# cviviers/graph-physics

Hardware: AMD Instinct MI355X
Metric: training-steps/sec + one-step velocity MSE, CylinderFlow MGN 15MP h=128 (higher is better)
Workload: dtype bf16; 1 GPU; CylinderFlow MGN 15MP h=128, batch=8 graphs per GPU (Cfg B); nodes_per_gpu=15384, edges_per_gpu=88560, global_batch=8, parallelism=dp1

## Files before the change

### graph-physics_amd/csrc/mgn_chain.h

```cpp
#pragma once
#include "mgn_common.h"

struct ChainFwdArgs {
    const __bf16* e;
    const __bf16* proj;
    const int32_t* proj_i;
    const int32_t* proj_j;
    const __bf16* wpack;
    int64_t woff[4];
    int32_t wks[4];
    const float* bias[4];
    const float* scale;
    float dinv;
    int64_t M, ntiles;
    __bf16* out;
    __bf16* z_save;
    float* rden_save;
    __bf16* act8;
    int64_t act_off[4];
    unsigned* mask32;
    int64_t mask_stride;
    float* agg_full;
    float* agg_head;
    float* agg_tail;
// ... 61 lines not shown
    float* rden_save;
    __bf16* act8;
    int64_t act_off[4];
    unsigned* mask32;
    int64_t mask_stride;
    const __bf16* pn_pack;
    const float* pn_b0;
    __bf16* pn_out;
    int32_t pn_kst;
    const float* agg_full;
    const float* agg_head;
    const float* agg_tail;
};

struct ChainNodeBwdArgs {
    const __bf16* dout;
    const __bf16* z_save;
    const float* rden_save;
    const float* scale;
    float dinv;
    const unsigned* mask32;
    int64_t mask_stride;
    const __bf16* wtpack;
    int64_t woff[4];
    int32_t wks[4];
    int64_t M, ntiles;
    __bf16* dz8;
    int64_t RP;
    float* dscale_part;
    __bf16* dx_part;
    __bf16* d_aggr;
};

bool chain_eligible(const mgn_mlp* m);
int chain16_edge_backward_parts(int64_t M);
int chain16_node_backward_parts(int64_t M);
bool chain_node_eligible(const mgn_mlp* m);
int chain16_node_forward(const mgn_mlp* m, const void* x, const mgn_topology* t, const mgn_mlp* edge,
                         const mgn_mlp_saved* edge_sv, int64_t M, void* x_out, void* aggr_save, mgn_mlp_saved* sv,
                         hipStream_t st, const mgn_mlp* next_edge = nullptr, void* next_proj = nullptr,
                         void* agg_scratch = nullptr);
size_t chain16_edge_agg_bytes(int64_t N, int64_t E);
int chain16_node_backward(const mgn_mlp* m, int64_t M, const mgn_mlp_saved* sv, const void* dout, void* dz8,
                          float* dscale_part, int* nparts, void* dx_part, void* d_aggr, hipStream_t st,
                          bool din2 = false);
int chain16_edge_forward(const mgn_mlp* m, const void* e, const void* proj, const int32_t* pi, const int32_t* pj,
                         int64_t M, void* out, mgn_mlp_saved* sv, hipStream_t st, bool z_p2, bool save_act = true,
                         int64_t N = 0, void* agg_scratch = nullptr);
int chain16_edge_wgrad_recompute(const mgn_mlp* m, const void* e, const void* proj, const int32_t* pi, const int32_t* pj,
                                 int64_t M, const void* dz8, float* part, int64_t G, int rows_per_chunk, int nchunks,
                                 hipStream_t st);
int chain16_edge_backward(const mgn_mlp* m, int64_t M, const mgn_mlp_saved* sv, const void* dout, const void* gath,
                          const int32_t* gath_idx, void* dz8, float* dscale_part, int* nparts, void* de, void* dz0,
                          hipStream_t st, bool p2, bool din2 = false, bool dout2 = false, int64_t N = 0,
                          void* agg_scratch = nullptr);
void chain16_edge_agg_parts(void* scratch, int64_t N, int64_t E, float** full, float** head, float** tail);
bool chain_dense_eligible(const mgn_mlp* m);
int chain16_dense_forward(const mgn_mlp* m, const void* in, int in_dtype, int64_t in_ld, const int32_t* in_rows,
                          int64_t M, void* out, int out_dtype, mgn_mlp_saved* sv, hipStream_t st);
int chain16_dense_backward(const mgn_mlp* m, int64_t M, const mgn_mlp_saved* sv, const void* dout, int dout_dtype,
                           void* din, int din_dtype, int64_t din_ld, void* dz8, float* dscale_part, int* nparts,
                           hipStream_t st);
```

### graph-physics_amd/csrc/mgn_chain16.hip

```cpp
#include <cmath>
#include <utility>
#include <cstring>
#include <mutex>
#include <type_traits>

#include "mgn_chain.h"
#include "mgn_chain16_dev.h"

#ifndef MGN_ABLATE
#define MGN_ABLATE 0
#endif
#ifndef MGN_DIRECT_ROWS
#define MGN_DIRECT_ROWS 0
#endif


#ifndef MGN_PROJ_HANDOFF
#define MGN_PROJ_HANDOFF 1
#endif

#ifndef MGN_BWD_HANDOFF
#define MGN_BWD_HANDOFF 1
#endif

// ... 1457 lines not shown
            relu_mask(acc, mcur[l - 1]);
            to_operand(acc, B);
        }
        store_r8(acc, scr, a.dz8, tile, lane);
        if (a.din) {
            f4 d2[2] = {f4{0.f, 0.f, 0.f, 0.f}, f4{0.f, 0.f, 0.f, 0.f}};
#pragma unroll
            for (int s = 0; s < 4; ++s)
#pragma unroll
                for (int t = 0; t < 2; ++t) d2[t] = mfma16(wfrag(W, 0, t, s, lane), B[s], d2[t]);
            if (ok) {
#pragma unroll
                for (int t = 0; t < 2; ++t)
#pragma unroll
                    for (int r = 0; r < 4; ++r) {
                        const int k = 16 * t + 4 * g + r;
                        if (k < a.K0) {
                            if (a.din_f32)
                                reinterpret_cast<float*>(a.din)[row * a.din_ld + k] = d2[t][r];
                            else
                                reinterpret_cast<__bf16*>(a.din)[row * a.din_ld + k] = (__bf16)d2[t][r];
                        }
                    }
            }
        }
        dpin<F32D>(nxt);
    }
    __syncthreads();
    if (threadIdx.x < H) {
        float s = 0.f;
#pragma unroll
        for (int w = 0; w < NW; ++w) s += red[w * H + threadIdx.x];
        a.dscale_part[(int64_t)blockIdx.x * H + threadIdx.x] = s;
    }
}

}

static size_t agg_al(size_t x) { return (x + 255) & ~(size_t)255; }
size_t chain16_edge_agg_bytes(int64_t N, int64_t E) {
    const int64_t nt = rows_pad(E) / TR;
    return agg_al((size_t)N * H * 4) + 2 * agg_al((size_t)nt * H * 4);
}
static void agg_carve(void* scratch, int64_t N, int64_t E, float** full, float** head, float** tail) {
    char* p = reinterpret_cast<char*>(scratch);
    *full = reinterpret_cast<float*>(p);
    p += agg_al((size_t)N * H * 4);
    *head = reinterpret_cast<float*>(p);
    p += agg_al((size_t)(rows_pad(E) / TR) * H * 4);
    *tail = reinterpret_cast<float*>(p);
}

void chain16_edge_agg_parts(void* scratch, int64_t N, int64_t E, float** full, float** head, float** tail) {
    agg_carve(scratch, N, E, full, head, tail);
}

int chain16_edge_forward(const mgn_mlp* m, const void* e, const void* proj, const int32_t* pi, const int32_t* pj,
                         int64_t M, void* out, mgn_mlp_saved* sv, hipStream_t st, bool z_p2, bool save_act, int64_t N,
                         void* agg_scratch) {
    ChainFwdArgs a;
    memset(&a, 0, sizeof(a));
    const bool eagg = agg_scratch != nullptr;
    if (eagg) agg_carve(agg_scratch, N, M, &a.agg_full, &a.agg_head, &a.agg_tail);
    a.e = reinterpret_cast<const __bf16*>(e);
    a.proj = reinterpret_cast<const __bf16*>(proj);
    a.proj_i = pi;
// ... 158 lines not shown

int chain16_node_backward(const mgn_mlp* m, int64_t M, const mgn_mlp_saved* sv, const void* dout, void* dz8,
                          float* dscale_part, int* nparts, void* dx_part, void* d_aggr, hipStream_t st, bool din2) {
    ChainNodeBwdArgs a;
    memset(&a, 0, sizeof(a));
    a.dout = reinterpret_cast<const __bf16*>(dout);
    a.z_save = reinterpret_cast<const __bf16*>(sv->z);
    a.rden_save = sv->rden;
    a.scale = m->scale;
    a.dinv = norm_dinv(m);
    a.mask32 = reinterpret_cast<const unsigned*>(sv->mask);
    a.mask_stride = mask_words_per_layer(*m, M);
    a.wtpack = reinterpret_cast<const __bf16*>(m->wtpack);
    layer_offsets(m, a.woff, a.wks);
    a.M = M;
    a.ntiles = rows_pad(M) / TR;
    a.dz8 = reinterpret_cast<__bf16*>(dz8);
    a.RP = rows_pad(M);
    a.dscale_part = dscale_part;
    a.dx_part = reinterpret_cast<__bf16*>(dx_part);
    a.d_aggr = reinterpret_cast<__bf16*>(d_aggr);
    *nparts = 0;
    if (M == 0) return 0;
    const auto kern = din2 ? chain16_node_bwd_kernel<true> : chain16_node_bwd_kernel<false>;
    if (int e2 = set_lds_once((const void*)kern, LDS_TOTAL)) return e2;
    const int grid = chain16_node_backward_parts(M);
    *nparts = grid;
    ProfScope ps(PROF_BWD_NODE, st);
    hipLaunchKernelGGL(kern, dim3(grid), dim3(NW * 64), LDS_TOTAL, st, a);
    MGN_LAUNCH_CHECK();
    return 0;
}

#ifndef MGN_CHAIN_DENSE
#define MGN_CHAIN_DENSE 1
#endif
bool chain_dense_eligible(const mgn_mlp* m) {
    return MGN_CHAIN_DENSE && m->dtype == MGN_BF16 && m->hidden == H && m->out_dim == H && m->n_layers == 4 &&
           m->has_norm && m->in_dim >= 1 && m->in_dim <= 32;
}

bool chain_eligible(const mgn_mlp* m) {
    return m->dtype == MGN_BF16 && m->hidden == H && m->in_dim == 3 * H && m->out_dim == H && m->n_layers == 4 &&
           m->has_norm;
}

int chain16_dense_forward(const mgn_mlp* m, const void* in, int in_dtype, int64_t in_ld, const int32_t* in_rows,
                          int64_t M, void* out, int out_dtype, mgn_mlp_saved* sv, hipStream_t st) {
    ChainDenseFwdArgs a;
    memset(&a, 0, sizeof(a));
    a.in = in;
    a.in_rows = in_rows;
    a.in_ld = in_ld;
    a.K0 = m->in_dim;
    a.in_f32 = in_dtype == MGN_F32;
    a.out_f32 = out_dtype == MGN_F32;
    a.wpack = reinterpret_cast<const __bf16*>(m->wpack);
    layer_offsets(m, a.woff, a.wks);
    for (int l = 0; l < 4; ++l) a.bias[l] = m->bias[l];
    a.scale = m->scale;
    a.dinv = norm_dinv(m);
    a.M = M;
    a.ntiles = rows_pad(M) / TR;
    a.out = out;
    a.z_save = reinterpret_cast<__bf16*>(sv->z);
    a.rden_save = sv->rden;
// ... 61 lines not shown
```

### graph-physics_amd/csrc/mgn_mlp.hip

```cpp
#include <vector>
#include <cstddef>
#include <cmath>
#include <cstdlib>
#include <cstring>
#include <mutex>
#include <unordered_map>

#include "mgn_chain.h"
#include "mgn_common.h"

namespace {

enum { MODE_DENSE = 0, MODE_EDGE = 1, MODE_NODE = 2 };

#ifdef MGN_STAMPS
#define F32C_STAMP_DECL unsigned long long st_prev = __builtin_amdgcn_s_memtime(), st_ph[12] = {0, 0, 0, 0, 0, 0, 0, 0, 0, 0, 0, 0}
#define F32C_STAMP(i)                                                                     \
    do {                                                                                  \
        __builtin_amdgcn_sched_barrier(0);                                                \
        unsigned long long st_t;                                                          \
        asm volatile("s_memtime %0\n\ts_waitcnt lgkmcnt(0)" : "=s"(st_t)::"memory");     \
        __builtin_amdgcn_sched_barrier(0);                                                \
        st_ph[i] += st_t - st_prev;                                                       \
        st_prev = st_t;                                                                   \
// ... 4042 lines not shown
    if (agg_scratch) {
        MGN_REQUIRE(!MGN_COMB_PAIR && H == 128 && sizeof(T) == 2, "edge-side aggregation: the chained bf16 blocks");
        float *full, *head, *tail;
        chain16_edge_agg_parts(agg_scratch, t->num_nodes, t->num_edges, &full, &head, &tail);
        a.agg_full = full;
        a.agg_head = head;
        a.agg_tail = tail;
    }
    a.dz0 = dz0;
    a.col_ptr = t->col_ptr;
    a.row_ptr = t->row_ptr;
    a.row_perm = t->row_perm;
    a.dx_part = dx_part;
    a.wt0 = edge->wtpack;
    a.dP8 = dP8;
    a.dx = dx;
    a.dx_pair = dx_pair && H == 128 && sizeof(T) == 2;
    a.N = t->num_nodes;
    a.RP = rows_pad(a.N);
    a.HP = rup(H, KSTEP);
    a.NS = cdiv(H, KSTEP);
    a.ldb = pad_ld<T>(2 * a.HP);
    const size_t lds = (size_t)BM * a.ldb * sizeof(T);
    auto fn = node_grad_kernel<T, H, BM>;
    if (int e = set_lds((const void*)fn, lds)) return e;
    const int grid = (int)(a.RP / BM);
    if (grid == 0) return 0;
    ProfScope ps(PROF_COMBINE, st);
    hipLaunchKernelGGL(fn, dim3(grid), dim3(MGN_THREADS), lds, st, a);
    MGN_LAUNCH_CHECK();
    return 0;
}

extern "C" {

int64_t mgn_linear_pack_elems(int32_t n, int32_t k, int32_t dtype) { return linear_pack_elems(n, k, dtype); }

int64_t mgn_mlp_pack_elems(const mgn_mlp* m) {
    int64_t t = 0;
    for (int l = 0; l < m->n_layers; ++l) {
        int n, k;
        mlp_layer_shape(*m, l, &n, &k);
        t += linear_pack_elems(n, k, m->dtype);
    }
    return t;
}

int mgn_pack_weights(const mgn_pack_job* jobs, int32_t njobs, int64_t max_elems, mgn_stream_t stream) {
    if (njobs <= 0) return 0;
    MGN_REQUIRE(jobs != nullptr, "pack jobs NULL");
    int64_t blocks = cdiv64(max_elems, 4 * MGN_THREADS);
    if (blocks > 1024) blocks = 1024;
    if (blocks < 1) blocks = 1;
    ProfScope ps(PROF_PACK, (hipStream_t)stream);
    hipLaunchKernelGGL(pack_kernel, dim3((unsigned)blocks, njobs), dim3(MGN_THREADS), 0, (hipStream_t)stream, jobs);
    MGN_LAUNCH_CHECK();
    return 0;
}

int mgn_mlp_forward(const mgn_mlp* m, const void* in, int32_t in_dtype, int64_t in_ld, const int32_t* in_rows,
                    int64_t rows, void* out, int32_t out_dtype, mgn_mlp_saved* saved, mgn_stream_t stream) {
    if (int e = check_mlp(m)) return e;
    MGN_REQUIRE(saved && saved->act && (m->n_layers < 2 || saved->mask) && (!m->has_norm || (saved->z && saved->rden)),
                "saved buffers missing");
    MGN_REQUIRE(in_dtype == MGN_F32 || in_dtype == m->dtype, "input dtype must be fp32 or the MLP dtype");
    if (chain_dense_eligible(m))
// ... 450 lines not shown
            return r;
    } else {
        MlpIn nin;
        memset(&nin, 0, sizeof(nin));
        nin.seg[0] = SrcSeg{x, nullptr, H, H, dt, 0, 0};
        nin.seg[1] = SrcSeg{saved->aggr, nullptr, H, H, dt, H, 0};
        nin.nseg = 2;
        BwdOut on;
        memset(&on, 0, sizeof(on));
        on.mode = MODE_NODE;
        on.o1 = c.dx_part;
        on.o2 = c.d_aggr;
        if (int r = mlp_backward_impl(node, MODE_NODE, t->num_nodes, nin, &saved->node, dx_out, dt, H, on, node_grads,
                                      c.mlp_ws, wl.nmlp - wl.mlp, st))
            return r;
    }
    const int64_t E = t->num_edges;
    BwdOut oe;
    memset(&oe, 0, sizeof(oe));
    oe.mode = MODE_EDGE;
    oe.gath = c.d_aggr;
    oe.gath_idx = t->csc_dst;
    oe.o1 = de;
    oe.o2 = c.dz0;
    if (chain_eligible(edge)) {
        int ntiles = 0;
        if (int r = chain16_edge_backward(edge, E, &saved->edge, de_out, c.d_aggr, t->csc_dst, c.dz8, c.dsp, &ntiles,
                                          de, c.dz0, st, chain_node_eligible(node), flags & MGN_BWD_DE_OUT_PAIR,
                                          flags & MGN_BWD_DE_PAIR, t->num_nodes, c.agg))
            return r;
    } else if (E > 0) {
        if (int r = mlp_bwd_any(edge, MODE_EDGE, E, &saved->edge, de_out, dt, H, oe, c.dz8, c.dsp, st)) return r;
    }
    int rc = 0;
    if (dt == MGN_F32) {
        MGN_DISPATCH_H(H, rc = (launch_node_grad<float, HH>(edge, t, c.dz0, c.dx_part, c.dP8, dx, st)))
    } else {
        MGN_DISPATCH_H(H, rc = (launch_node_grad<__bf16, HH>(edge, t, c.dz0, c.dx_part, c.dP8, dx, st,
                                                              flags & MGN_BWD_DX_PAIR, c.agg)))
    }
    return rc;
}

int mgn_block_backward_data(const mgn_topology* t, const mgn_mlp* edge, const mgn_mlp* node, const void* x,
                            const void* e, const mgn_block_saved* saved, const void* dx_out, const void* de_out,
                            void* dx, void* de, float* edge_grads, float* node_grads, void* ws, size_t ws_bytes,
                            mgn_stream_t stream) {
    (void)e;
    (void)edge_grads;
    return block_backward_data_impl(t, edge, node, x, saved, dx_out, de_out, dx, de, node_grads, ws, ws_bytes,
                                    nullptr, stream);
}

static int block_backward_wgrad_impl(const mgn_topology* t, const mgn_mlp* edge, const mgn_mlp* node, const void* x,
                                     const void* e, const mgn_block_saved* saved, const void* de_out,
                                     float* edge_grads, float* node_grads, void* ws, size_t ws_bytes, void* keep,
                                     RedDesc* defer, mgn_stream_t stream) {
    BlockWs wl;
    if (int r = block_bwd_check(t, edge, node, de_out, ws_bytes, &wl)) return r;
    hipStream_t st = (hipStream_t)stream;
    const int H = edge->hidden, dt = edge->dtype;
    const BlockBwdCarve c = block_bwd_carve(t, edge, node, ws, wl, keep);
    const int64_t E = t->num_edges, N = t->num_nodes;
    if (c.chained) {
        BlockWgradIn in;
        in.E = E;
        in.N = N;
        in.e = e;
        in.x = x;
        in.aggr = saved->aggr;
        in.eact = saved->edge.act;
        in.edz8 = c.dz8;
        in.dz0 = c.dz0;
        in.dP8 = c.dP8;
// ... 118 lines not shown
        if (int r = block_backward_data_impl(t, edge, node, x, saved, dx_out, de_out, dx, de, node_grads, ws,
                                             ws_bytes, nullptr, stream, flags))
            return r;
        return block_backward_wgrad_impl(t, edge, node, x, e, saved, de_out, edge_grads, node_grads, ws, ws_bytes,
                                         nullptr, nullptr, stream);
    }
    MGN_REQUIRE(keep_bytes >= keep_layout(t, edge, node).total, "block backward keep buffer too small");
    if (part != MGN_BWD_WGRAD_ONLY) {
        if (int r = block_backward_data_impl(t, edge, node, x, saved, dx_out, de_out, dx, de, node_grads, ws, ws_bytes,
                                             keep, stream, flags))
            return r;
        if (part == MGN_BWD_DATA_ONLY) return 0;
    }
    RedDesc d[2];
    memset(d, 0, sizeof(d));
    if (int r = block_backward_wgrad_impl(t, edge, node, x, e, saved, de_out, edge_grads, node_grads, ws, ws_bytes,
                                          keep, d, stream))
        return r;
    memcpy(reduce2, d, sizeof(d));
    return 0;
}

int mgn_block_backward_deferred3(const mgn_topology* t, const mgn_mlp* edge, const mgn_mlp* node, const void* x,
                                 const void* e, const mgn_block_saved* saved, const void* dx_out, const void* de_out,
                                 void* dx, void* de, float* edge_grads, float* node_grads, void* ws,
                                 size_t ws_bytes, void* keep, size_t keep_bytes, mgn_wgrad_reduce* reduce2,
                                 int32_t flags, const mgn_call_opts* opts, mgn_stream_t stream) {
    MGN_REQUIRE(!opts || (opts->data_cus >= 0 && opts->wgrad_cus >= 0), "CU caps must be >= 0 (0 = no cap)");
    CallScope cs(opts);
    return mgn_block_backward_deferred2(t, edge, node, x, e, saved, dx_out, de_out, dx, de, edge_grads, node_grads, ws,
                                        ws_bytes, keep, keep_bytes, reduce2, flags, stream);
}

int mgn_wgrad_reduce_many(const mgn_wgrad_reduce* reds, int32_t n, mgn_stream_t stream) {
    MGN_REQUIRE(n >= 0 && (n == 0 || reds), "bad reduction list");
    std::vector<RedDesc> d;
    for (int32_t i = 0; i < n; ++i) {
        RedDesc x;
        memcpy(&x, &reds[i], sizeof(x));
        if (x.blocks > 0) d.push_back(x);
    }
    if (d.empty()) return 0;
    return launch_reduce2(d.data(), (int)d.size(), (hipStream_t)stream);
}

int mgn_block_backward(const mgn_topology* t, const mgn_mlp* edge, const mgn_mlp* node, const void* x, const void* e,
                       const mgn_block_saved* saved, const void* dx_out, const void* de_out, void* dx, void* de,
                       float* edge_grads, float* node_grads, void* ws, size_t ws_bytes, mgn_stream_t stream) {
    if (int r = mgn_block_backward_data(t, edge, node, x, e, saved, dx_out, de_out, dx, de, edge_grads, node_grads,
                                        ws, ws_bytes, stream))
        return r;
    return mgn_block_backward_wgrad(t, edge, node, x, e, saved, dx_out, de_out, dx, de, edge_grads, node_grads, ws,
                                    ws_bytes, stream);
}

}
```

### graph-physics_amd/graphphysics/_native.py

```python
import ctypes
import os

import torch

LIB_PATH = os.path.join(os.path.dirname(os.path.abspath(__file__)), "_lib", "libmgn.so")
ABI_VERSION = 17

MGN_F32 = 0
MGN_BF16 = 1
MGN_BWD_DE_OUT_PAIR = 1
MGN_BWD_DE_PAIR = 2
MGN_BWD_DX_OUT_PAIR = 4
MGN_BWD_DX_PAIR = 8
MGN_BWD_DATA_ONLY = 16
MGN_BWD_WGRAD_ONLY = 32
MGN_MAX_LAYERS = 8

_vp = ctypes.c_void_p
_i32 = ctypes.c_int32
_i64 = ctypes.c_int64
_sz = ctypes.c_size_t
_dbl = ctypes.c_double
_f32 = ctypes.c_float
_u32 = ctypes.c_uint32
# ... 90 lines not shown
    "mgn_block_forward_chain": (_i32, [ctypes.POINTER(Topology), ctypes.POINTER(Mlp), ctypes.POINTER(Mlp),
                                       _vp, _vp, _vp, _vp, ctypes.POINTER(BlockSaved), _vp, _sz, _i32,
                                       ctypes.POINTER(Mlp), _vp, _sz, ctypes.POINTER(ctypes.c_int32), _vp]),
    "mgn_block_forward_scratch_bytes": (_sz, [ctypes.POINTER(Topology), ctypes.POINTER(Mlp), ctypes.POINTER(Mlp)]),
    "mgn_block_forward_chain2": (_i32, [ctypes.POINTER(Topology), ctypes.POINTER(Mlp), ctypes.POINTER(Mlp),
                                        _vp, _vp, _vp, _vp, ctypes.POINTER(BlockSaved), _vp, _sz, _i32,
                                        ctypes.POINTER(Mlp), _vp, _sz, ctypes.POINTER(ctypes.c_int32), _vp, _sz, _vp]),
    "mgn_block_backward_workspace_bytes": (_sz, [ctypes.POINTER(Topology), ctypes.POINTER(Mlp),
                                                 ctypes.POINTER(Mlp)]),
    "mgn_block_backward": (_i32, [ctypes.POINTER(Topology), ctypes.POINTER(Mlp), ctypes.POINTER(Mlp),
                                  _vp, _vp, ctypes.POINTER(BlockSaved), _vp, _vp, _vp, _vp, _vp, _vp,
                                  _vp, _sz, _vp]),
    "mgn_block_backward_data": (_i32, [ctypes.POINTER(Topology), ctypes.POINTER(Mlp), ctypes.POINTER(Mlp),
                                       _vp, _vp, ctypes.POINTER(BlockSaved), _vp, _vp, _vp, _vp, _vp, _vp,
                                       _vp, _sz, _vp]),
    "mgn_block_backward_wgrad": (_i32, [ctypes.POINTER(Topology), ctypes.POINTER(Mlp), ctypes.POINTER(Mlp),
                                        _vp, _vp, ctypes.POINTER(BlockSaved), _vp, _vp, _vp, _vp, _vp, _vp,
                                        _vp, _sz, _vp]),
    "mgn_block_backward_keep_bytes": (_sz, [ctypes.POINTER(Topology), ctypes.POINTER(Mlp), ctypes.POINTER(Mlp)]),
    "mgn_block_backward_deferred": (_i32, [ctypes.POINTER(Topology), ctypes.POINTER(Mlp), ctypes.POINTER(Mlp),
                                           _vp, _vp, ctypes.POINTER(BlockSaved), _vp, _vp, _vp, _vp, _vp, _vp,
                                           _vp, _sz, _vp, _sz, ctypes.POINTER(WgradReduce), _vp]),
    "mgn_block_backward_deferred2": (_i32, [ctypes.POINTER(Topology), ctypes.POINTER(Mlp), ctypes.POINTER(Mlp),
                                            _vp, _vp, ctypes.POINTER(BlockSaved), _vp, _vp, _vp, _vp, _vp, _vp,
                                            _vp, _sz, _vp, _sz, ctypes.POINTER(WgradReduce), _i32, _vp]),
    "mgn_wgrad_reduce_many": (_i32, [ctypes.POINTER(WgradReduce), _i32, _vp]),
    "mgn_block_backward_deferred3": (_i32, [ctypes.POINTER(Topology), ctypes.POINTER(Mlp), ctypes.POINTER(Mlp),
                                            _vp, _vp, ctypes.POINTER(BlockSaved), _vp, _vp, _vp, _vp, _vp, _vp,
                                            _vp, _sz, _vp, _sz, ctypes.POINTER(WgradReduce), _i32,
                                            ctypes.POINTER(CallOpts), _vp]),
    "mgn_mlp_backward_deferred3": (_i32, [ctypes.POINTER(Mlp), _vp, _i32, _i64, _vp, _i64,
                                          ctypes.POINTER(MlpSaved), _vp, _i32, _vp, _i32, _vp, _vp, _sz, _vp, _sz,
                                          ctypes.POINTER(WgradReduce), _i32, ctypes.POINTER(CallOpts), _vp]),
    "mgn_debug_wave_times": (_i32, [_i32, _vp, _i32]),
    "mgn_graph_attention_workspace_bytes": (_sz, [ctypes.POINTER(Topology), _i32, _i32, _i32]),
    "mgn_graph_attention_forward": (_i32, [ctypes.POINTER(Topology), _vp, _vp, _vp, _i64, _i32, _i32, _i32, _vp,
                                           _vp, _vp]),
    "mgn_graph_attention_backward": (_i32, [ctypes.POINTER(Topology), _vp, _vp, _vp, _vp, _vp, _vp, _i64, _i32,
                                            _i32, _i32, _vp, _vp, _vp, _vp, _sz, _vp]),
    "mgn_gated_mlp_row_tile": (_i32, []),
    "mgn_gated_mlp_blocks": (_i32, [_i64, _i32]),
    "mgn_gated_mlp_saved_bytes": (_sz, [ctypes.POINTER(GatedMlp), _i64]),
    "mgn_gated_mlp_forward": (_i32, [ctypes.POINTER(GatedMlp), _vp, _i64, _i64, _vp, _i64, _vp, _vp]),
    "mgn_gated_mlp_backward_workspace_bytes": (_sz, [ctypes.POINTER(GatedMlp), _i64]),
    "mgn_gated_mlp_backward": (_i32, [ctypes.POINTER(GatedMlp), _vp, _i64, _i64, _vp, _vp, _i64, _vp, _vp, _vp, _sz,
                                      _vp]),
    "mgn_permute_rows": (_i32, [_vp, _vp, _vp, _i64, _i32, _i32, _i32, _i32, _vp]),
    "mgn_segment_sum": (_i32, [_vp, _vp, _i64, _i32, _i32, _vp, _vp]),
    "mgn_column_stats_workspace_bytes": (_sz, [_i64, _i32]),
    "mgn_column_stats": (_i32, [_vp, _i64, _i32, _i64, _vp, _vp, _sz, _vp]),
    "mgn_normalizer_workspace_bytes": (_sz, [_i64, _i32]),
    "mgn_normalizer_forward": (_i32, [_vp, _i64, _i32, _i64, _i32, _vp, _vp, _vp, _vp, _vp, _f32, _f32, _vp,
                                      _vp, _sz, _vp]),
    "mgn_simulator_preamble_workspace_bytes": (_sz, [_i64, _i64]),
    "mgn_simulator_preamble": (_i32, [_vp, _i64, _i64, _i32, _i32, _i32, _i32, _i32, _i32, _vp, _i64, _vp, _i64,
                                      _i32, _i64, _i32, ctypes.POINTER(NormalizerState),
                                      ctypes.POINTER(NormalizerState), ctypes.POINTER(NormalizerState), _vp, _vp,
                                      _vp, _vp, _vp, _sz, _vp]),
    "mgn_simulator_statistics": (_i32, [_vp, _i64, _i64, _i32, _i32, _i32, _i32, _i32, _i32, _vp, _i64, _vp, _i64,
                                        _i32, _i64, _vp, _vp, _vp, _sz, _vp]),
    "mgn_masked_mse_workspace_bytes": (_sz, [_i64]),
    "mgn_masked_mse": (_i32, [_vp, _vp, _i64, _i32, _vp, _i64, _u32, _vp, _vp, _vp, _vp, _sz, _vp]),
    "mgn_masked_mse_backward": (_i32, [_vp, _vp, _i64, _i32, _vp, _i64, _u32, _vp, _vp, _vp, _vp]),
    "mgn_gmm_nll_workspace_bytes": (_sz, [_i64]),
    "mgn_gmm_nll_diag": (_i32, [_vp, _vp, _i64, _i32, _i32, _f32, _vp, _i64, _u32, _vp, _vp, _vp, _vp, _sz, _vp]),
    "mgn_gmm_nll_diag_backward": (_i32, [_vp, _vp, _i64, _i32, _i32, _f32, _vp, _i64, _u32, _vp, _vp, _vp, _vp]),
# ... 204 lines not shown


def require_device(t):
    if not t.is_cuda:
        raise RuntimeError("the MI355X MGN path needs tensors on a HIP device (no CPU fallback)")


def stream_ptr(device=None):
    return _vp(torch.cuda.current_stream(device).cuda_stream)


def ptr(t):
    if t is None:
        return _vp(0)
    if isinstance(t, _vp):
        return t
    if isinstance(t, int):
        return _vp(t)
    return _vp(t.data_ptr())


def mgn_dtype(torch_dtype):
    if torch_dtype == torch.float32:
        return MGN_F32
    if torch_dtype == torch.bfloat16:
        return MGN_BF16
    raise ValueError(f"unsupported compute dtype {torch_dtype}")


def torch_dtype(mdt):
    return torch.float32 if mdt == MGN_F32 else torch.bfloat16


def column_stats(x):
    import torch

    require_device(x)
    if x.dtype != torch.float32 or x.dim() != 2 or x.stride(1) != 1:
        x = x.float().contiguous()
    rows, cols = x.shape
    out = torch.empty(2 * cols, dtype=torch.float32, device=x.device)
    ws = torch.empty(max(int(lib().mgn_column_stats_workspace_bytes(rows, cols)), 4), dtype=torch.uint8,
                     device=x.device)
    check(lib().mgn_column_stats(ptr(x), rows, cols, x.stride(0), ptr(out), ptr(ws), ws.numel(),
                                 stream_ptr(x.device)))
    return out[:cols].view(1, cols), out[cols:].view(1, cols)


def normalizer_state(n, accumulate):
    pend = n._pending_packed if accumulate else None
    return NormalizerState(n._acc_sum.data_ptr(), n._acc_sum_squared.data_ptr(), n._acc_count.data_ptr(),
                           n._num_accumulations.data_ptr(), pend.data_ptr() if pend is not None else None,
                           float(n._max_accumulations), n._eps())


def simulator_preamble(x, y, edge_attr, feat, out, type_index, n_types, accumulate, out_norm, node_norm,
                       edge_norm):
    import torch

    require_device(x)
    N, E = x.shape[0], (edge_attr.shape[0] if edge_norm is not None else 0)
    dev = x.device
    to = torch.empty((N, out[1] - out[0]), dtype=torch.float32, device=dev)
    no = torch.empty((N, feat[1] - feat[0] + n_types), dtype=torch.float32, device=dev)
    eo = torch.empty((E, edge_attr.shape[1]), dtype=torch.float32, device=dev) if edge_norm is not None else None
    ws = torch.empty(int(lib().mgn_simulator_preamble_workspace_bytes(N, E)), dtype=torch.uint8, device=dev)
# ... 486 lines not shown
```

### include/mgn.h

```cpp
#ifndef MGN_H
#define MGN_H

#include <stddef.h>
#include <stdint.h>

#ifdef __cplusplus
extern "C" {
#endif

typedef struct ihipStream_t* mgn_stream_t;

#define MGN_ABI_VERSION 17
#define MGN_F32 0
#define MGN_BF16 1
#define MGN_MAX_LAYERS 8

int mgn_abi_version(void);
const char* mgn_last_error(void);

#define MGN_ERR_EDGE_INDEX 1u
#define MGN_ERR_TYPE_NEG 2u
#define MGN_ERR_TYPE_BIG 4u
#define MGN_ERR_HANDOFF 8u
#define MGN_ERR_WORLD_CAPACITY 16u
// ... 123 lines not shown
#define MGN_BWD_DX_OUT_PAIR 4
#define MGN_BWD_DX_PAIR 8
#define MGN_BWD_DATA_ONLY 16
#define MGN_BWD_WGRAD_ONLY 32
int mgn_block_backward_deferred2(const mgn_topology* t, const mgn_mlp* edge, const mgn_mlp* node,
                                 const void* x, const void* e, const mgn_block_saved* saved,
                                 const void* dx_out, const void* de_out, void* dx, void* de,
                                 float* edge_grads, float* node_grads, void* ws, size_t ws_bytes,
                                 void* keep, size_t keep_bytes, mgn_wgrad_reduce* reduce2,
                                 int32_t flags, mgn_stream_t stream);
int mgn_wgrad_reduce_many(const mgn_wgrad_reduce* reds, int32_t n, mgn_stream_t stream);
int mgn_mlp_backward_deferred2(const mgn_mlp* m, const void* in, int32_t in_dtype, int64_t in_ld,
                               const int32_t* in_rows, int64_t rows, const mgn_mlp_saved* saved,
                               const void* dout, int32_t dout_dtype, void* din, int32_t din_dtype,
                               float* grads, void* ws, size_t ws_bytes, void* keep, size_t keep_bytes,
                               mgn_wgrad_reduce* reduce1, int32_t flags, mgn_stream_t stream);
typedef struct mgn_call_opts {
    int32_t data_cus;
    int32_t wgrad_cus;
    uint32_t* err_word;
} mgn_call_opts;
int mgn_block_backward_deferred3(const mgn_topology* t, const mgn_mlp* edge, const mgn_mlp* node,
                                 const void* x, const void* e, const mgn_block_saved* saved,
                                 const void* dx_out, const void* de_out, void* dx, void* de,
                                 float* edge_grads, float* node_grads, void* ws, size_t ws_bytes,
                                 void* keep, size_t keep_bytes, mgn_wgrad_reduce* reduce2,
                                 int32_t flags, const mgn_call_opts* opts, mgn_stream_t stream);
int mgn_mlp_backward_deferred3(const mgn_mlp* m, const void* in, int32_t in_dtype, int64_t in_ld,
                               const int32_t* in_rows, int64_t rows, const mgn_mlp_saved* saved,
                               const void* dout, int32_t dout_dtype, void* din, int32_t din_dtype,
                               float* grads, void* ws, size_t ws_bytes, void* keep, size_t keep_bytes,
                               mgn_wgrad_reduce* reduce1, int32_t flags, const mgn_call_opts* opts,
                               mgn_stream_t stream);
int mgn_debug_wave_times(int32_t kind, uint64_t* out, int32_t n);
size_t mgn_mlp_backward_keep_bytes(const mgn_mlp* m, int64_t rows);
int mgn_mlp_backward_deferred(const mgn_mlp* m, const void* in, int32_t in_dtype, int64_t in_ld,
                              const int32_t* in_rows, int64_t rows, const mgn_mlp_saved* saved,
                              const void* dout, int32_t dout_dtype, void* din, int32_t din_dtype,
                              float* grads, void* ws, size_t ws_bytes, void* keep, size_t keep_bytes,
                              mgn_wgrad_reduce* reduce1, mgn_stream_t stream);
int mgn_block_backward_data(const mgn_topology* t, const mgn_mlp* edge, const mgn_mlp* node,
                            const void* x, const void* e, const mgn_block_saved* saved,
                            const void* dx_out, const void* de_out, void* dx, void* de,
                            float* edge_grads, float* node_grads, void* ws, size_t ws_bytes,
                            mgn_stream_t stream);
int mgn_block_backward_wgrad(const mgn_topology* t, const mgn_mlp* edge, const mgn_mlp* node,
                             const void* x, const void* e, const mgn_block_saved* saved,
                             const void* dx_out, const void* de_out, void* dx, void* de,
                             float* edge_grads, float* node_grads, void* ws, size_t ws_bytes,
                             mgn_stream_t stream);

#define MGN_HAS_GRAPH_ATTENTION 1
size_t mgn_graph_attention_workspace_bytes(const mgn_topology* t, int32_t hidden, int32_t heads, int32_t dtype);
int mgn_graph_attention_forward(const mgn_topology* t, const void* q, const void* k, const void* v,
                                int64_t ld, int32_t hidden, int32_t heads, int32_t dtype,
                                void* y, float* lse , mgn_stream_t stream);
int mgn_graph_attention_backward(const mgn_topology* t, const void* q, const void* k, const void* v,
                                 const void* y, const float* lse, const void* dy, int64_t ld,
                                 int32_t hidden, int32_t heads, int32_t dtype,
                                 void* dq, void* dk, void* dv, void* ws, size_t ws_bytes, mgn_stream_t stream);

int mgn_permute_rows(const void* in, void* out, const int32_t* idx, int64_t rows, int32_t cols,
                     int32_t in_dtype, int32_t out_dtype, int32_t scatter, mgn_stream_t stream);
int mgn_segment_sum(const void* src, const int32_t* seg_ptr, int64_t segments, int32_t cols,
                    int32_t dtype, void* out, mgn_stream_t stream);

// ... 243 lines not shown
```

Baseline: 352.5 steps/s.

## Add fused chained node-gradient kernel combining CSR gather-sum with MFMA projection

Adds a new HIP kernel for the node-gradient step of the message-passing block backward. Each wave gathers and sums edge dz0 rows per node over the column CSR and the permuted row CSR. It converts the two sums to MFMA operands, multiplies them by the edge layer-0 transposed weights staged in LDS, adds dx_part and writes dx, and also stores the summed dP8 tiles. The generic launch_node_grad path is still used when the edge MLP is not bf16 with h=128, when edge-side aggregation scratch is present, or when the graph is small or dense. The aim is to cut the separate launches and the global round trips of the generic path. The cost is extra register pressure from the 8-row gather unroll and LDS staging.

```diff
diff --git a/graph-physics_amd/csrc/mgn_chain.h b/graph-physics_amd/csrc/mgn_chain.h
--- a/graph-physics_amd/csrc/mgn_chain.h
+++ b/graph-physics_amd/csrc/mgn_chain.h
@@ -117,7 +117,22 @@
     __bf16* d_aggr;
 };
 
+struct ChainNodeGradArgs {
+    const __bf16* dz0;
+    const int32_t* col_ptr;
+    const int32_t* row_ptr;
+    const int32_t* row_perm;
+    const __bf16* dx_part;
+    const __bf16* wt;
+    __bf16* dP8;
+    __bf16* dx;
+    int64_t N, RP, ntiles;
+};
+
 bool chain_eligible(const mgn_mlp* m);
+bool chain_node_grad_eligible(const mgn_mlp* edge);
+int chain16_node_grad(const mgn_mlp* edge, const mgn_topology* t, const void* dz0, const void* dx_part, void* dP8,
+                      void* dx, bool dx_pair, hipStream_t st);
 int chain16_edge_backward_parts(int64_t M);
 int chain16_node_backward_parts(int64_t M);
 bool chain_node_eligible(const mgn_mlp* m);
diff --git a/graph-physics_amd/csrc/mgn_chain16.hip b/graph-physics_amd/csrc/mgn_chain16.hip
--- a/graph-physics_amd/csrc/mgn_chain16.hip
+++ b/graph-physics_amd/csrc/mgn_chain16.hip
@@ -1513,6 +1513,188 @@
 #pragma unroll
         for (int w = 0; w < NW; ++w) s += red[w * H + threadIdx.x];
         a.dscale_part[(int64_t)blockIdx.x * H + threadIdx.x] = s;
+    }
+}
+
+#ifndef MGN_NG_SG
+#define MGN_NG_SG 8
+#endif
+constexpr int NG_SG = MGN_NG_SG;
+constexpr int NG_WELEMS = 2 * LFR * FRAG;
+constexpr size_t NG_LDS_W = (size_t)NG_WELEMS * 2;
+constexpr int NG_SROWS = SROWS + TR;
+constexpr size_t NG_LDS = NG_LDS_W + (size_t)NW * NG_SROWS * SLD * 2;
+
+__device__ __forceinline__ void ng_rows(u32x4 (&t)[NG_SG][4], const __bf16* dz, const int (&id)[NG_SG], int g) {
+#pragma unroll
+    for (int u = 0; u < NG_SG; ++u)
+#pragma unroll
+        for (int s = 0; s < 4; ++s)
+            t[u][s] = *reinterpret_cast<const u32x4*>(dz + (int64_t)id[u] * H + 32 * s + 8 * g);
+}
+
+__device__ __forceinline__ void ng_add(float (&acc)[4][8], const u32x4 (&t)[NG_SG][4], int k, int ke) {
+#pragma unroll
+    for (int u = 0; u < NG_SG; ++u)
+        if (k + u < ke) {
+#pragma unroll
+            for (int s = 0; s < 4; ++s) {
+                const bf16x8 v = __builtin_bit_cast(bf16x8, t[u][s]);
+#pragma unroll
+                for (int e = 0; e < 8; ++e) acc[s][e] += (float)v[e];
+            }
+        }
+}
+
+__device__ __forceinline__ void ng_operand(const float (&acc)[4][8], bf16x8 (&B)[4], int lane) {
+    const int from = 4 * (4 * (lane & 15) + (lane >> 4));
+#pragma unroll
+    for (int s = 0; s < 4; ++s) {
+        bf16x8 v;
+#pragma unroll
+        for (int e = 0; e < 8; ++e) v[e] = (__bf16)acc[s][e];
+        u32x4 w = __builtin_bit_cast(u32x4, v);
+#pragma unroll
+        for (int i = 0; i < 4; ++i) w[i] = (unsigned)__builtin_amdgcn_ds_bpermute(from, (int)w[i]);
+        B[s] = __builtin_bit_cast(bf16x8, w);
+    }
+}
+
+__device__ __forceinline__ void ng_store_r8(const bf16x8 (&B)[4], __bf16* scr, __bf16* dst, int64_t tile, int lane) {
+    const int m = lane & 15, g = lane >> 4;
+#pragma unroll
+    for (int u = 0; u < 2; ++u) {
+        if ((m >> 3) == u) {
+#pragma unroll
+            for (int s = 0; s < 4; ++s) *reinterpret_cast<bf16x8*>(scr + (m & 7) * SLD + 32 * s + 8 * g) = B[s];
+        }
+        lds_fence();
+        unsigned rv[8];
+#pragma unroll
+        for (int q = 0; q < 8; ++q) rv[q] = *reinterpret_cast<const unsigned*>(scr + q * SLD + 2 * lane);
+        bf16x8 c0, c1;
+#pragma unroll
+        for (int q = 0; q < 8; ++q) {
+            const bf16x2 p = __builtin_bit_cast(bf16x2, rv[q]);
+            c0[q] = p[0];
+            c1[q] = p[1];
+        }
+        __bf16* p = dst + (((int64_t)tile * 2 + u) * H + 2 * lane) * 8;
+        *reinterpret_cast<bf16x8*>(p) = c0;
+        *reinterpret_cast<bf16x8*>(p + 8) = c1;
+        lds_fence();
+    }
+}
+
+template <bool P2>
+__global__ __launch_bounds__(NW * 64) void chain16_node_grad_kernel(ChainNodeGradArgs a) {
+    extern __shared__ __attribute__((aligned(16))) char smem[];
+    __bf16* W = reinterpret_cast<__bf16*>(smem);
+    const int lane = threadIdx.x & 63, wave = __builtin_amdgcn_readfirstlane(threadIdx.x >> 6);
+    __bf16* scr = reinterpret_cast<__bf16*>(smem + NG_LDS_W) + wave * NG_SROWS * SLD;
+    __bf16* dxs = scr + SROWS * SLD;
+    const int m = lane & 15, g = lane >> 4;
+    const int sm = lane >> 2, sg = lane & 3;
+    const int64_t stride = (int64_t)gridDim.x * NW;
+    int64_t tile = (int64_t)wave * gridDim.x + blockIdx.x;
+    bf16x8 Bi[4], Bj[4];
+    auto stage = [&]() {
+#pragma unroll
+        for (int i = 0; i < NG_WELEMS / FRAG / NW; ++i) {
+            const int pc = wave + i * NW;
+            __builtin_amdgcn_global_load_lds(
+                (const __attribute__((address_space(1))) void*)(a.wt + pc * FRAG + lane * 8),
+                (__attribute__((address_space(3))) void*)(W + pc * FRAG), 16, 0, 0);
+        }
+    };
+    auto gather = [&](int64_t tl, auto stage_tag) {
+        const int g = sg;
+        const int64_t v = tl * TR + sm;
+        const bool ok = v < a.N;
+        const int64_t vr = clamp_row(v, a.N);
+        int kb0 = a.col_ptr[vr], ke0 = a.col_ptr[vr + 1], kb1 = a.row_ptr[vr], ke1 = a.row_ptr[vr + 1];
+        ke0 = ok ? ke0 : kb0;
+        ke1 = ok ? ke1 : kb1;
+        u32x4 dxl[4];
+#pragma unroll
+        for (int p = 0; p < 4; ++p)
+            dxl[p] = *reinterpret_cast<const u32x4*>(a.dx_part + clamp_row(tl * TR + 4 * p + (lane >> 4), a.N) * H +
+                                                     8 * (lane & 15));
+        int id[NG_SG];
+        u32x4 rows[NG_SG][4];
+        if (kb1 < ke1) {
+#pragma unroll
+            for (int u = 0; u < NG_SG; ++u) id[u] = a.row_perm[kb1 + u < ke1 ? kb1 + u : ke1 - 1];
+        }
+        if (kb0 < ke0) {
+            int k0[NG_SG];
+#pragma unroll
+            for (int u = 0; u < NG_SG; ++u) k0[u] = kb0 + u < ke0 ? kb0 + u : ke0 - 1;
+            ng_rows(rows, a.dz0, k0, g);
+        }
+        if constexpr (decltype(stage_tag)::value) stage();
+        float acc[4][8];
+#pragma unroll
+        for (int s = 0; s < 4; ++s)
+#pragma unroll
+            for (int e = 0; e < 8; ++e) acc[s][e] = 0.f;
+#pragma unroll
+        for (int p = 0; p < 4; ++p)
+            *reinterpret_cast<u32x4*>(dxs + (4 * p + (lane >> 4)) * SLD + 8 * (lane & 15)) = dxl[p];
+        if (kb0 < ke0) {
+            ng_add(acc, rows, kb0, ke0);
+#pragma unroll 1
+            for (int k = kb0 + NG_SG; k < ke0; k += NG_SG) {
+                int kk[NG_SG];
+#pragma unroll
+                for (int u = 0; u < NG_SG; ++u) kk[u] = k + u < ke0 ? k + u : ke0 - 1;
+                ng_rows(rows, a.dz0, kk, g);
+                ng_add(acc, rows, k, ke0);
+            }
+        }
+        ng_operand(acc, Bi, lane);
+#pragma unroll
+        for (int s = 0; s < 4; ++s)
+#pragma unroll
+            for (int e = 0; e < 8; ++e) acc[s][e] = 0.f;
+        if (kb1 < ke1) {
+#pragma unroll 1
+            for (int k = kb1; k < ke1; k += NG_SG) {
+                ng_rows(rows, a.dz0, id, g);
+#pragma unroll
+                for (int u = 0; u < NG_SG; ++u) id[u] = a.row_perm[k + NG_SG + u < ke1 ? k + NG_SG + u : ke1 - 1];
+                ng_add(acc, rows, k, ke1);
+            }
+        }
+        ng_operand(acc, Bj, lane);
+    };
+    if (tile < a.ntiles)
+        gather(tile, std::true_type{});
+    else
+        stage();
+    asm volatile("s_waitcnt vmcnt(0)" ::: "memory");
+    __syncthreads();
+    while (tile < a.ntiles) {
+        ng_store_r8(Bi, scr, a.dP8, tile, lane);
+        ng_store_r8(Bj, scr, a.dP8 + a.RP * H, tile, lane);
+        f4 acc[8];
+#pragma unroll
+        for (int t = 0; t < 8; ++t) acc[t] = f4{0.f, 0.f, 0.f, 0.f};
+#pragma unroll
+        for (int b = 0; b < 2; ++b)
+#pragma unroll
+            for (int s = 0; s < 4; ++s) {
+#pragma unroll
+                for (int t = 0; t < 8; ++t)
+                    acc[t] = mfma16(*reinterpret_cast<const bf16x8*>(W + ((size_t)((b * 8 + t) * 4 + s) * 64 + lane) * 8),
+                                    b ? Bj[s] : Bi[s], acc[t]);
+                __builtin_amdgcn_sched_barrier(0);
+            }
+#pragma unroll
+        for (int t = 0; t < 8; ++t) acc[t] += bf4(*reinterpret_cast<const u32x2*>(dxs + m * SLD + 16 * t + 4 * g));
+        store_rows<P2>(acc, scr, a.dx, tile, a.N, lane);
+        tile += stride;
+        if (tile < a.ntiles) gather(tile, std::false_type{});
     }
 }
 
@@ -1737,6 +1919,34 @@
     return 0;
 }
 
+bool chain_node_grad_eligible(const mgn_mlp* edge) {
+    return edge->dtype == MGN_BF16 && edge->hidden == H && edge->in_dim == 3 * H && edge->wtpack != nullptr;
+}
+
+int chain16_node_grad(const mgn_mlp* edge, const mgn_topology* t, const void* dz0, const void* dx_part, void* dP8,
+                      void* dx, bool dx_pair, hipStream_t st) {
+    ChainNodeGradArgs a;
+    memset(&a, 0, sizeof(a));
+    a.dz0 = reinterpret_cast<const __bf16*>(dz0);
+    a.col_ptr = t->col_ptr;
+    a.row_ptr = t->row_ptr;
+    a.row_perm = t->row_perm;
+    a.dx_part = reinterpret_cast<const __bf16*>(dx_part);
+    a.wt = reinterpret_cast<const __bf16*>(edge->wtpack) + (int64_t)LFR * FRAG;
+    a.dP8 = reinterpret_cast<__bf16*>(dP8);
+    a.dx = reinterpret_cast<__bf16*>(dx);
+    a.N = t->num_nodes;
+    a.RP = rows_pad(a.N);
+    a.ntiles = a.RP / TR;
+    if (a.ntiles == 0) return 0;
+    const auto kern = dx_pair ? chain16_node_grad_kernel<true> : chain16_node_grad_kernel<false>;
+    if (int e2 = set_lds_once((const void*)kern, NG_LDS)) return e2;
+    ProfScope ps(PROF_COMBINE, st);
+    hipLaunchKernelGGL(kern, dim3(node_grid(a.ntiles)), dim3(NW * 64), NG_LDS, st, a);
+    MGN_LAUNCH_CHECK();
+    return 0;
+}
+
 #ifndef MGN_CHAIN_DENSE
 #define MGN_CHAIN_DENSE 1
 #endif
diff --git a/graph-physics_amd/csrc/mgn_mlp.hip b/graph-physics_amd/csrc/mgn_mlp.hip
--- a/graph-physics_amd/csrc/mgn_mlp.hip
+++ b/graph-physics_amd/csrc/mgn_mlp.hip
@@ -4098,6 +4098,27 @@
     return 0;
 }
 
+#ifndef MGN_CHAIN_NODE_GRAD
+#define MGN_CHAIN_NODE_GRAD 1
+#endif
+constexpr int64_t NODE_GRAD_MIN_N = 8192;
+static int node_grad_any(const mgn_mlp* edge, const mgn_topology* t, const void* dz0, const void* dx_part, void* dP8,
+                         void* dx, hipStream_t st, bool dx_pair, void* agg_scratch, int impl) {
+    const int H = edge->hidden;
+    const bool can = chain_node_grad_eligible(edge) && agg_scratch == nullptr;
+    MGN_REQUIRE(impl != 2 || can, "chained node_grad: bf16 h=128 edge MLP without edge-side aggregation only");
+    const bool pays = t->num_nodes >= NODE_GRAD_MIN_N && t->num_edges <= 8 * t->num_nodes;
+    if (impl == 2 || (impl == 0 && MGN_CHAIN_NODE_GRAD && can && pays))
+        return chain16_node_grad(edge, t, dz0, dx_part, dP8, dx, dx_pair, st);
+    int rc = 0;
+    if (edge->dtype == MGN_F32) {
+        MGN_DISPATCH_H(H, rc = (launch_node_grad<float, HH>(edge, t, dz0, dx_part, dP8, dx, st)))
+    } else {
+        MGN_DISPATCH_H(H, rc = (launch_node_grad<__bf16, HH>(edge, t, dz0, dx_part, dP8, dx, st, dx_pair, agg_scratch)))
+    }
+    return rc;
+}
+
 extern "C" {
 
 int64_t mgn_linear_pack_elems(int32_t n, int32_t k, int32_t dtype) { return linear_pack_elems(n, k, dtype); }
@@ -4614,14 +4635,7 @@
     } else if (E > 0) {
         if (int r = mlp_bwd_any(edge, MODE_EDGE, E, &saved->edge, de_out, dt, H, oe, c.dz8, c.dsp, st)) return r;
     }
-    int rc = 0;
-    if (dt == MGN_F32) {
-        MGN_DISPATCH_H(H, rc = (launch_node_grad<float, HH>(edge, t, c.dz0, c.dx_part, c.dP8, dx, st)))
-    } else {
-        MGN_DISPATCH_H(H, rc = (launch_node_grad<__bf16, HH>(edge, t, c.dz0, c.dx_part, c.dP8, dx, st,
-                                                              flags & MGN_BWD_DX_PAIR, c.agg)))
-    }
-    return rc;
+    return node_grad_any(edge, t, c.dz0, c.dx_part, c.dP8, dx, st, flags & MGN_BWD_DX_PAIR, c.agg, 0);
 }
 
 int mgn_block_backward_data(const mgn_topology* t, const mgn_mlp* edge, const mgn_mlp* node, const void* x,
@@ -4806,6 +4820,19 @@
                                         ws_bytes, keep, keep_bytes, reduce2, flags, stream);
 }
 
+int mgn_node_grad(const mgn_topology* t, const mgn_mlp* edge, const void* dz0, const void* dx_part, void* dP8,
+                  void* dx, int32_t dx_pair, int32_t impl, const mgn_call_opts* opts, mgn_stream_t stream) {
+    MGN_REQUIRE(t && edge, "topology and edge MLP required");
+    MGN_REQUIRE(!opts || (opts->data_cus >= 0 && opts->wgrad_cus >= 0), "CU caps must be >= 0 (0 = no cap)");
+    MGN_REQUIRE(impl >= 0 && impl <= 2, "impl: 0 auto, 1 generic, 2 chained");
+    MGN_REQUIRE(edge->dtype == MGN_F32 || edge->dtype == MGN_BF16, "unsupported dtype");
+    MGN_REQUIRE(edge->in_dim == 3 * edge->hidden && edge->wtpack, "edge MLP of a block: layer 0 is [h x 3h], packed");
+    MGN_REQUIRE(!dx_pair || (edge->dtype == MGN_BF16 && edge->hidden == 128), "pair-layout dx: bf16 h=128 only");
+    MGN_REQUIRE(t->num_nodes == 0 || ((dz0 || t->num_edges == 0) && dx_part && dP8 && dx), "node_grad buffers NULL");
+    CallScope cs(opts);
+    return node_grad_any(edge, t, dz0, dx_part, dP8, dx, (hipStream_t)stream, dx_pair != 0, nullptr, impl);
+}
+
 int mgn_wgrad_reduce_many(const mgn_wgrad_reduce* reds, int32_t n, mgn_stream_t stream) {
     MGN_REQUIRE(n >= 0 && (n == 0 || reds), "bad reduction list");
     std::vector<RedDesc> d;
diff --git a/graph-physics_amd/graphphysics/_native.py b/graph-physics_amd/graphphysics/_native.py
--- a/graph-physics_amd/graphphysics/_native.py
+++ b/graph-physics_amd/graphphysics/_native.py
@@ -146,6 +146,8 @@
     "mgn_mlp_backward_deferred3": (_i32, [ctypes.POINTER(Mlp), _vp, _i32, _i64, _vp, _i64,
                                           ctypes.POINTER(MlpSaved), _vp, _i32, _vp, _i32, _vp, _vp, _sz, _vp, _sz,
                                           ctypes.POINTER(WgradReduce), _i32, ctypes.POINTER(CallOpts), _vp]),
+    "mgn_node_grad": (_i32, [ctypes.POINTER(Topology), ctypes.POINTER(Mlp), _vp, _vp, _vp, _vp, _i32, _i32,
+                             ctypes.POINTER(CallOpts), _vp]),
     "mgn_debug_wave_times": (_i32, [_i32, _vp, _i32]),
     "mgn_graph_attention_workspace_bytes": (_sz, [ctypes.POINTER(Topology), _i32, _i32, _i32]),
     "mgn_graph_attention_forward": (_i32, [ctypes.POINTER(Topology), _vp, _vp, _vp, _i64, _i32, _i32, _i32, _vp,
@@ -416,6 +418,16 @@
     return torch.float32 if mdt == MGN_F32 else torch.bfloat16
 
 
+NODE_GRAD_AUTO, NODE_GRAD_GENERIC, NODE_GRAD_CHAINED = 0, 1, 2
+
+
+def node_grad(topo, edge, dz0, dx_part, dP8, dx, dx_pair=False, impl=NODE_GRAD_AUTO, data_cus=0):
+    require_device(dx)
+    opts = CallOpts(int(data_cus), 0, None)
+    check(lib().mgn_node_grad(ctypes.byref(topo), ctypes.byref(edge), ptr(dz0), ptr(dx_part), ptr(dP8), ptr(dx),
+                              int(bool(dx_pair)), int(impl), ctypes.byref(opts), stream_ptr(dx.device)))
+
+
 def column_stats(x):
     import torch
 
diff --git a/include/mgn.h b/include/mgn.h
--- a/include/mgn.h
+++ b/include/mgn.h
@@ -179,6 +179,10 @@
                                float* grads, void* ws, size_t ws_bytes, void* keep, size_t keep_bytes,
                                mgn_wgrad_reduce* reduce1, int32_t flags, const mgn_call_opts* opts,
                                mgn_stream_t stream);
+#define MGN_HAS_NODE_GRAD 1
+int mgn_node_grad(const mgn_topology* t, const mgn_mlp* edge, const void* dz0, const void* dx_part,
+                  void* dP8, void* dx, int32_t dx_pair, int32_t impl, const mgn_call_opts* opts,
+                  mgn_stream_t stream);
 int mgn_debug_wave_times(int32_t kind, uint64_t* out, int32_t n);
 size_t mgn_mlp_backward_keep_bytes(const mgn_mlp* m, int64_t rows);
 int mgn_mlp_backward_deferred(const mgn_mlp* m, const void* in, int32_t in_dtype, int64_t in_ld,
```

After: 356.6 steps/s, median of 6. 1.01x the previous value.
